# BogdanDIA/gr-dvbt

Hardware: AMD Instinct MI355X
Metric: RX Msamples/s (baseband in -> TS out) (higher is better)
Workload: dtype u8 (Viterbi/RS) + f32 (front end)

## Files before the change

gr_dvbt_amd/csrc/k_backend.hpp:

```cpp
#pragma once
#include <hip/hip_runtime.h>
#include <stdint.h>
#include "k_frontend.hpp"

namespace dvbt {

struct InnerParams { int payload, m, csize; int nlev; float inv_step, guard; float hshift; int hier; };
__device__ __forceinline__ float hier_unshift(float x, float hshift) { return copysignf(fmaxf(fabsf(x) - hshift, 0.f), x); }

__device__ __forceinline__ int demap_all(float2 v, const float2 *pts, int csize)
{
  float dr = v.x - pts[0].x, di = v.y - pts[0].y;
  float best = dr * dr + di * di; int idx = 0;
  for (int j = 1; j < csize; j++) {
    dr = v.x - pts[j].x; di = v.y - pts[j].y;
    float d = dr * dr + di * di;
    if (d < best) { best = d; idx = j; }
  }
  return idx;
}

__device__ __forceinline__ int demap_fast(float2 v, const float2 *pts, const unsigned char *label_of, const InnerParams &p)
{
  const bool in_range = p.nlev != 0 && fabsf(v.x) < p.guard && fabsf(v.y) < p.guard;
// ... 60 lines not shown
    const uint8_t *bb = v + blk * 132;
    auto bit = [&](int f) -> int { const int e = f / 126, j = f - e * 126; int w = j - offs[e]; if (w < 0) w += 126; return (bb[w] >> (m - 1 - e)) & 1; };
    const int t0 = m * i;
    const int hp = (bit((t0 & 1) * 126 + t0 / 2) << 1) | bit(((t0 + 1) & 1) * 126 + (t0 + 1) / 2);
    int lp = 0;
    for (int k = 2; k < m - 2; k++) {
      const int t = t0 + k, e = (t % (m - 2)) / ((m - 2) / 2) + 2 * (t % ((m - 2) / 2)) + 2, f = e * 126 + t / (m - 2);
      lp = (lp << 1) | (f < m * 126 ? bit(f) : 0);
    }
    o_hp[idx] = (uint8_t)hp;
    if (o_lp) o_lp[idx] = (uint8_t)lp;
  }
}

constexpr int INNER_NB = 12;
constexpr int INNER_THREADS = DVBT_INNER_THREADS;
template <int MODE> __global__ __launch_bounds__(INNER_THREADS) void inner_kernel(const float2 *__restrict__ eq, const uint8_t *__restrict__ in_bytes, InnerParams p,
                                                   const RxState *st, int nitems_fixed, const int *__restrict__ sym_index,
                                                   const float2 *__restrict__ points, const unsigned char *__restrict__ label_tab,
                                                   const uint16_t *__restrict__ H, const uint16_t *__restrict__ Hinv,
                                                   uint8_t *__restrict__ tap_demap, uint8_t *__restrict__ tap_symdeint,
                                                   uint8_t *__restrict__ out, uint8_t *__restrict__ out_lp = nullptr)
{
  extern __shared__ __attribute__((aligned(16))) unsigned char smem_raw[];
  uint8_t *v = smem_raw;
  float2 *pts = reinterpret_cast<float2 *>(smem_raw + ((((p.payload + IB - 1) / IB) * IBS + 15) & ~15));
  unsigned char *label_of = reinterpret_cast<unsigned char *>(pts + 64);
  const int u = blockIdx.x, tid = threadIdx.x;
  constexpr int mode = MODE;
  int first = 0, nout = nitems_fixed;
  if (st) { first = st->first_out; nout = st->n_out_symbols; if (first < 0) return; }
  if (u >= nout) return;
  const int s = first + u;
  if (mode & 1) {
    for (int j = tid; j < p.csize; j += INNER_THREADS) pts[j] = points[j];
    if (tid < 64) label_of[tid] = label_tab[tid];
  }
  __syncthreads();
  const bool odd = (mode & 2) ? (sym_index[s] & 1) : false;
  const float2 *e = eq ? eq + (size_t)s * p.payload : nullptr;
  const uint8_t *ib = in_bytes ? in_bytes + (size_t)s * p.payload : nullptr;
  const uint16_t *ptab = odd ? H : Hinv;
  for (int q0 = tid; q0 < p.payload; q0 += INNER_NB * INNER_THREADS) {
    unsigned pk[INNER_NB];
#pragma unroll
    for (int k = 0; k < INNER_NB; k++) {
      const int q = q0 + k * INNER_THREADS, qc = q < p.payload ? q : p.payload - 1;
      pk[k] = (mode & 2) ? (unsigned)ptab[qc] : (unsigned)qc;
      if (!(mode & 1)) pk[k] |= (unsigned)ib[qc] << 16;
    }
#pragma unroll
    for (int k = 0; k < INNER_NB; k++) {
      const int q = q0 + k * INNER_THREADS;
      if (q < p.payload) {
        const int lab = (mode & 1) ? demap_one(e[q], pts, label_of, p) : (int)(pk[k] >> 16);
        const int dst = (int)(pk[k] & 0xffffu);
        const int blk = dst / IB, r = dst - blk * IB, at = blk * IBS + r;
        v[at] = (uint8_t)lab;
        if (r < IBS - IB) v[at + IB] = (uint8_t)lab;
        if (tap_demap && (mode & 1)) tap_demap[(size_t)u * p.payload + q] = (uint8_t)lab;
      }
    }
  }
  __syncthreads();
  uint8_t *o = out + (size_t)u * p.payload;
  if (tap_symdeint) for (int q = tid; q < p.payload; q += INNER_THREADS) tap_symdeint[(size_t)u * p.payload + q] = v[ipos(q)];
  if (!(mode & 4)) { for (int q = tid; q < p.payload; q += INNER_THREADS) o[q] = v[ipos(q)]; return; }
  if (p.hier) bit_deint_hier(v, o, out_lp ? out_lp + (size_t)u * p.payload : nullptr, p.payload, p.m, tid);
  else if (p.m == 2) bit_deint_words<2>(v, o, p.payload, tid);
  else if (p.m == 4) bit_deint_words<4>(v, o, p.payload, tid);
  else bit_deint_words<6>(v, o, p.payload, tid);
}

struct VitParams {
  int m, k, n, plen, ntb, bsize;
  int d_nsymbols;
  int d_nbits;
  int chunk_bytes;
  int payload;
  unsigned punct_mask;
  int warm;
  unsigned long long prefix_nib;
  unsigned long long magic_plen, magic_m;
  unsigned long long punct_rep;
  unsigned magic16_plen;
  uint8_t punct[16], prefix[16];
};

__device__ __forceinline__ void plan_body(RxState *st, const VitParams &vp, long long sym_off)
{
  const long long ibits = (long long)vp.payload * vp.m * vp.k / vp.n;
  const long long nin_g = (sym_off + (long long)st->n_out_symbols) * vp.payload;
  const long long nblocks_g = nin_g / vp.d_nsymbols;
  long long nin = nblocks_g * vp.d_nsymbols - sym_off * vp.payload;
  long long steps = nblocks_g * (vp.d_nbits / 2) - sym_off * ibits;
  if (nin < 0 || steps < 0) { nin = 0; steps = 0; }
  st->n_vit_in = nin;
  st->n_vit_steps = steps;
  long long nb_g = nblocks_g * (vp.d_nbits / 2) / 8 - vp.ntb;
  if (nb_g < 0) nb_g = 0;
  long long nb = steps / 8 - vp.ntb;
  if (nb < 0) nb = 0;
  st->n_vit_bytes = nb;
  const long long items_g = (nb_g / 1632) & ~1ll;
  long long words = items_g * 8 - sym_off * ibits / (8 * 204);
  if (words < 0) words = 0;
  st->stream_rs_items = items_g;
  st->n_rs_words = words;
  st->n_rs_items = words / 8;
  st->sym_off = sym_off;
  st->n_ts_bytes = 0; st->rs_fail = 0; st->rs_corr = 0; st->ts_first_packet = 0; st->rs_list_n = 0;
}
__global__ __launch_bounds__(256) void tps_tail_kernel(FrontParams p, RxState *st, const SymInfo *info, const int *maj, TpsState *ts, int *sym_index,
                                                      const TpsEdge *edges, const int *first_cand, int *need_seq, int clear_d_init, VitParams vp, long long sym_off)
{
  int seq = 1;
  if (edges) seq = tps_finalize_body(st, edges, first_cand, need_seq, p.keep_last, ts);
  if (seq) tps_fsm_body(p, st, 0, info, maj, ts, sym_index, (int *)nullptr, (const unsigned char *)nullptr, clear_d_init);
  if (threadIdx.x == 0) plan_body(st, vp, sym_off);
}

struct RsTables { const uint8_t *div_tab;  const uint8_t *gexp;  const uint8_t *glog;  };

constexpr int RS_SYN_STRIDE = 65;
__device__ inline int rs_decode_word_wave(uint8_t *cw, const uint8_t *syn, const uint8_t *gexp, const uint8_t *glog,
                                          int compat, uint8_t *scr, int lane)
{
  auto gmul = [&](int a, int b) -> int { return (a == 0 || b == 0) ? 0 : gexp[glog[a] + glog[b]]; };
  auto gdiv = [&](int a, int b) -> int { return (a == 0 || b == 0) ? 0 : gexp[255 + glog[a] - glog[b]]; };
  auto wxor = [&](int v) -> int { for (int o = 16; o > 0; o >>= 1) v ^= __shfl_xor(v, o); return v; };
  int sig = lane == 0 ? 1 : 0, bb = sig, el = 0;
  for (int r = 1; r <= 16; r++) {
    int term = (lane < r && lane <= 16) ? gmul(sig, syn[(r - 1 - lane) * RS_SYN_STRIDE]) : 0;
    const int discr = __shfl(wxor(term), 0);
    int bup = __shfl_up(bb, 1); if (lane == 0) bup = 0;
    if (discr == 0) bb = bup;
    else {
      const int T = sig ^ gmul(discr, bup);
      if (2 * el <= r - 1) { el = r - el; bb = gdiv(sig, discr); } else bb = bup;
      sig = lane <= 16 ? T : 0;
    }
  }
  const unsigned long long nz = __ballot(sig != 0 && lane <= 16);
  const int deg_sigma = nz ? 63 - __clzll(nz) : 0;
  uint8_t *s_sig = scr, *s_root = scr + 17, *s_om = scr + 34;
  if (lane <= 16) s_sig[lane] = (uint8_t)sig;
  __builtin_amdgcn_fence(__ATOMIC_SEQ_CST, "wavefront");
  int found[4]; int nroots = 0;
  unsigned long long bal[4];
  for (int k = 0; k < 4; k++) {
    const int i = lane + 1 + 64 * k;
    int q = 1;
    if (i <= 255) {
      for (int j = 1; j <= deg_sigma; j++) { int sg = s_sig[j]; if (sg) q ^= gexp[(glog[sg] + (j * i) % 255) % 255]; }
    }
    found[k] = (i <= 255) && (q == 0);
    bal[k] = __ballot(found[k]);
  }
  {
    int before = 0;
    for (int k = 0; k < 4; k++) {
      if (found[k]) { int rank = before + __popcll(bal[k] & ((1ull << lane) - 1)); if (rank < 17 && rank < deg_sigma) s_root[rank] = (uint8_t)(lane + 1 + 64 * k); }
      before += __popcll(bal[k]);
    }
    nroots = before < deg_sigma ? before : deg_sigma;
  }
// ... 410 lines not shown
```

gr_dvbt_amd/csrc/k_viterbi3.hpp:

```cpp
#pragma once
#include <hip/hip_runtime.h>
#include <stdint.h>
#include <limits.h>
#include <string.h>
#include "dvbt_tables.hpp"
#include "k_backend.hpp"

namespace dvbt {

inline VitParams make_vit_params(const Dims &d, int bsize, int chunk_bytes)
{
  VitParams v; memset(&v, 0, sizeof v);
  v.m = d.m; v.k = d.k; v.n = d.n; v.plen = d.plen; v.ntb = d.ntb; v.bsize = bsize;
  v.d_nsymbols = bsize * d.n / d.m; v.d_nbits = 2 * d.k * bsize;
  v.chunk_bytes = chunk_bytes > 0 ? chunk_bytes : 768; v.payload = d.payload; v.warm = 72;
  memcpy(v.punct, d.punct, 16); memcpy(v.prefix, d.prefix, 16);
  v.punct_mask = 0; v.prefix_nib = 0;
  for (int i = 0; i < d.plen; i++) { v.punct_mask |= (unsigned)d.punct[i] << i; v.prefix_nib |= (unsigned long long)d.prefix[i] << (4 * i); }
  v.magic_plen = ~0ull / (unsigned)d.plen + 1; v.magic_m = ~0ull / (unsigned)d.m + 1;
  for (int i = 0; i < 64; i++) v.punct_rep |= (unsigned long long)d.punct[i % d.plen] << i;
  v.magic16_plen = (65536u + (unsigned)d.plen - 1) / (unsigned)d.plen;
  return v;
}

#define DPP_XOR1 0xB1
#define DPP_XOR2 0x4E
#define DPP_HALF_MIRROR 0x141
#define DPP_ROR8 0x128
#define DPP_MIRROR 0x140

__device__ __forceinline__ int rotl6(int c, int p) { return ((c << p) | (c >> (6 - p))) & 63; }

#ifndef V3_WGW_N
#define V3_WGW_N 4
#endif
constexpr int V3_WGW = V3_WGW_N;
#ifndef V3_EXP
#define V3_EXP 0
#endif
constexpr int V3_WARM = 72;
constexpr int V3_WARM_MAX = 1152;
static_assert(V3_WARM == 72, "make_vit_params (above) presets VitParams.warm to the default");
constexpr int V3_BLK = 24;
constexpr int V3_RENORM_EVERY = 6;
constexpr int V3_RENORM_BEST = -72;
static_assert(V3_BLK % V3_RENORM_EVERY == 0, "a block of windows ends right behind a renormalisation: equal states are equal registers at a block's top (proof, repair, carried state)");
static_assert(V3_RENORM_BEST % 2 == 0, "the renormalisation leaves bit 8 of the cells alone");
static_assert(V3_RENORM_BEST - 49 - 4 >= -128, "lowest candidate of a step: the best field never decreases, the spread is at most 49, |delta| <= 4");
static_assert(V3_RENORM_BEST + 1 + 4 * 8 * V3_RENORM_EVERY + 4 <= 127, "highest candidate of a step: the best field rises by at most 4 per step, 8 steps per window");
constexpr int V3_RINGW = 64;
constexpr int V3_WAVES_PER_CU = 4 * 2;
constexpr int V3_CBW = 17;

typedef short v3pk __attribute__((ext_vector_type(2)));
__device__ __forceinline__ v3pk pk(int x) { return __builtin_bit_cast(v3pk, x); }
__device__ __forceinline__ int ipk(v3pk x) { return __builtin_bit_cast(int, x); }
__device__ __forceinline__ int pk_add(int a, int b) { return ipk(pk(a) + pk(b)); }
__device__ __forceinline__ int pk_sub(int a, int b) { return ipk(pk(a) - pk(b)); }
__device__ __forceinline__ int pk_max(int a, int b) { return ipk(__builtin_elementwise_max(pk(a), pk(b))); }
__device__ __forceinline__ int pk_min(int a, int b) { return ipk(__builtin_elementwise_min(pk(a), pk(b))); }
template <int CTRL> __device__ __forceinline__ int dppb(int v) { return __builtin_amdgcn_update_dpp(0, v, CTRL, 0xf, 0xf, true); }
__device__ __forceinline__ int vconst(int c) { int x; asm("v_mov_b32 %0, %1" : "=v"(x) : "s"(c)); return x; }
__device__ __forceinline__ int pk_max_swap(int a, int b) { int r; asm("v_pk_max_i16 %0, %1, %2 op_sel:[0,1] op_sel_hi:[1,0]" : "=v"(r) : "v"(a), "v"(b)); return r; }
template <bool HI> __device__ __forceinline__ int pk_add_half(int a, int b)
{
  int r;
  if (HI) asm("v_pk_add_u16 %0, %1, %2 op_sel:[0,1] op_sel_hi:[1,1]" : "=v"(r) : "v"(a), "v"(b));
  else asm("v_pk_add_u16 %0, %1, %2 op_sel:[0,0] op_sel_hi:[1,0]" : "=v"(r) : "v"(a), "v"(b));
  return r;
}
template <bool HI> __device__ __forceinline__ int pk_sub_half(int a, int b)
{
  int r;
  if (HI) asm("v_pk_sub_i16 %0, %1, %2 op_sel:[0,1] op_sel_hi:[1,1]" : "=v"(r) : "v"(a), "v"(b));
  else asm("v_pk_sub_i16 %0, %1, %2 op_sel:[0,0] op_sel_hi:[1,0]" : "=v"(r) : "v"(a), "v"(b));
  return r;
}

struct V3Lane {
  unsigned sel[6];
  int bias8[6][2];
  int kc[3][2];
  int org[2];
  int arm_mid[3][2];
  int arm_b2[3][2];
  int arm_org[3][2];
};

__device__ __forceinline__ int v3_phys(int a) { const int a2 = (a >> 2) & 1; return (a & 8) | (a2 << 2) | ((a & 3) ^ (a2 ? 3 : 0)); }
__device__ __forceinline__ int v3_log(int p) { const int q = p & 7, a2 = (q >> 2) & 1; return (p & 8) | (a2 << 2) | ((q ^ (a2 ? 7 : 0)) & 3); }
__device__ __forceinline__ int v3_cell_of_z(int z) { return ((z & 2) << 4) | ((z & 1) << 4) | v3_log(z >> 2); }
__device__ __forceinline__ int v3_z_of_cell(int c) { return v3_phys(c & 15) * 4 + ((c >> 5) & 1) * 2 + ((c >> 4) & 1); }

__device__ __forceinline__ int v3_upper(int P, int r, int h, int a) { const int c = (r << 5) | (h << 4) | a; return (c >> (5 - P)) & 1; }
__device__ __forceinline__ unsigned v3_class(int P, int r, int h, int a)
{
  const int c = (r << 5) | (h << 4) | a, i = rotl6(c, P) & 31;
  const int c0 = ((i >> 2) ^ (i >> 1) ^ i) & 1;
  const int c1 = ((i >> 4) ^ (i >> 2) ^ (i >> 1)) & 1;
  return (unsigned)(c0 | (c1 << 1));
}
__device__ inline void v3_init_lane(int pl, V3Lane &L)
// ... 120 lines not shown
__device__ __forceinline__ void v3_trace_out(const V3Trace &T, const unsigned char *tab, uint8_t *outb) { unsigned t[2]; v3_trace_read(T, tab, t); v3_trace_store<false>(T, t, outb); }

__device__ __forceinline__ void v3_load_words(const unsigned *wp_, unsigned (&W)[8])
{
  const uint4 *wp = reinterpret_cast<const uint4 *>(wp_);
  const uint4 t0 = wp[0], t1 = wp[1];
  W[0] = t0.x; W[1] = t0.y; W[2] = t0.z; W[3] = t0.w; W[4] = t1.x; W[5] = t1.y; W[6] = t1.z; W[7] = t1.w;
}
template <int V6, int W0, bool HOPS, int HOP0, int NTB, int NW, bool PREF> __device__ __forceinline__ void v3_fwd_window(int (&v)[2], const V3Lane &L, const unsigned *wrow, unsigned char *tab, unsigned char *tabw,
                                                                                           unsigned char *bests, int jb, int dd, int pl, V3Trace &T, unsigned (&W)[8], unsigned (&Wn)[8], uint8_t *outb)
{
  constexpr bool HOPA = HOPS && HOP0 + 2 * V6 < NTB - 1, HOPB = HOPS && HOP0 + 2 * V6 + 1 < NTB - 1;
  constexpr bool FINA = HOPS && HOP0 + 2 * V6 == NTB - 1, FINB = HOPS && HOP0 + 2 * V6 + 1 == NTB - 1;
  unsigned th[2], tout[2];
  if (HOPA) v3_hop_read(T, tab, th);
  if (FINA) v3_trace_read(T, tab, tout);
  constexpr int WB = W0 + V6;
  static_assert(V3_BLK % 8 == 0 && V3_RINGW % 8 == 0, "jb % 8 == 0: the ring's wrap falls between two groups of eight windows");
  const int jr = ((jb + (WB & ~7)) & (V3_RINGW - 1)) + (WB & 7);
#if V3_EXP & 256
  for (int i = 0; i < 8; i++) { W[i] = (unsigned)((jb + W0) * 0x01010101 + i * 0x00020406 + pl); asm volatile("" : "+v"(W[i])); }
#else
  if (PREF) v3_load_words(wrow + (V6 + 1) * 8, Wn);
#endif
  constexpr int P0 = (8 * V6) % 6;
  int raw[2];
#if V3_EXP & 32
  if (V6 & 1) __builtin_amdgcn_s_setprio(1); else __builtin_amdgcn_s_setprio(0);
#endif
#if V3_EXP & 128
  __builtin_amdgcn_s_sleep(1);
#endif
  v3_step<(P0 + 0) % 6, 0>(v, W[0], L, raw); V3_YIELD(); v3_step<(P0 + 1) % 6, 0>(v, W[1], L, raw); V3_YIELD(); v3_step<(P0 + 2) % 6, 3>(v, W[2], L, raw); V3_YIELD();
  if (HOPA) { v3_hop_merge<NW>(T, th); if (HOPB) v3_hop_read(T, tab, th); }
  if (FINB) v3_trace_read(T, tab, tout);
  if (FINA) v3_trace_store<true>(T, tout, outb);
  v3_step<(P0 + 3) % 6, 0>(v, W[3], L, raw); V3_YIELD(); v3_step<(P0 + 4) % 6, 0>(v, W[4], L, raw); V3_YIELD(); v3_step<(P0 + 5) % 6, 1>(v, W[5], L, raw); V3_YIELD();
  v3_step<(P0 + 6) % 6, 4>(v, W[6], L, raw); V3_YIELD(); v3_step<(P0 + 7) % 6, 2>(v, W[7], L, raw);
  if (HOPB) v3_hop_merge<NW>(T, th);
  if (FINB) v3_trace_store<true>(T, tout, outb);
  if (!(V3_EXP & 4)) *reinterpret_cast<unsigned *>(tabw + jr * V3_ROW<NW>) = __builtin_amdgcn_perm((unsigned)raw[1], (unsigned)raw[0], 0x06040200u);
  if (V3_EXP & 2) { if (raw[0] == 0x12345) bests[jr] = 1; return; }
  const int s = v3_window_end<(P0 + 2) % 6, V6 == V3_RENORM_EVERY - 1>(v, L);
  bests[dd * V3_RINGW + jr] = (unsigned char)s;
}
static_assert(V3_RENORM_EVERY == 6, "v3_fwd_six is the group of windows that ends in a renormalisation (V6 = 0..5)");
template <int W0, bool HOPS, int HOP0, int NTB, int NW, bool MORE> __device__ __forceinline__ void v3_fwd_six(int (&v)[2], const V3Lane &L, const unsigned *wrow, unsigned char *tab, unsigned char *tabw,
                                                                                  unsigned char *bests, int jb, int dd, int pl, V3Trace &T, unsigned (&Wa)[8], unsigned (&Wb)[8], uint8_t *outb)
{
  v3_fwd_window<0, W0, HOPS, HOP0, NTB, NW, true>(v, L, wrow, tab, tabw, bests, jb, dd, pl, T, Wa, Wb, outb); v3_fwd_window<1, W0, HOPS, HOP0, NTB, NW, true>(v, L, wrow, tab, tabw, bests, jb, dd, pl, T, Wb, Wa, outb);
  v3_fwd_window<2, W0, HOPS, HOP0, NTB, NW, true>(v, L, wrow, tab, tabw, bests, jb, dd, pl, T, Wa, Wb, outb); v3_fwd_window<3, W0, HOPS, HOP0, NTB, NW, true>(v, L, wrow, tab, tabw, bests, jb, dd, pl, T, Wb, Wa, outb);
  v3_fwd_window<4, W0, HOPS, HOP0, NTB, NW, true>(v, L, wrow, tab, tabw, bests, jb, dd, pl, T, Wa, Wb, outb); v3_fwd_window<5, W0, HOPS, HOP0, NTB, NW, MORE>(v, L, wrow, tab, tabw, bests, jb, dd, pl, T, Wb, Wa, outb);
}

#if V3_EXP & 16
__device__ unsigned long long *v3_dbg;
#endif

constexpr int V3_SLOT = 32;
constexpr int V3_CTL_CHUNKS = 0;
constexpr int V3_CTL_MISMATCH = 1;
constexpr int V3_CTL_CONFLICT = 2;
constexpr int V3_CTL_UNPROVEN = 3;
constexpr int V3_CTL_SEQ = 4;
constexpr int V3_CTL_ACC = 8;
constexpr int V3_CTL_SHORT = 12;
constexpr int V3_CTL_HDR = 16;
struct V3Aux {
  int *snap;
  int *ctl;
  long long cap;
  long long grid0;
  const int *carry_in;
  int *carry_out; int carry_rel;
  int debug;
};
constexpr int V3_DEBUG_WALK = 2;
__device__ __forceinline__ int *v3_own(const V3Aux &ax, long long c) { return ax.snap + (3 * c) * V3_SLOT; }
__device__ __forceinline__ int *v3_pred(const V3Aux &ax, long long c) { return ax.snap + (3 * c + 1) * V3_SLOT; }
__device__ __forceinline__ int *v3_fix(const V3Aux &ax, long long c) { return ax.snap + (3 * c + 2) * V3_SLOT; }
inline size_t v3_snap_words(long long cap) { return (size_t)(cap + 2) * 3 * V3_SLOT; }
inline size_t v3_ctl_words(long long cap) { return (size_t)V3_CTL_HDR + 2 * (size_t)(cap + 2); }

struct V3Lds { unsigned char *tab; unsigned *wbuf; unsigned char *bests; const unsigned *lut; int wv; };
__device__ __forceinline__ void v3_init_lut(unsigned *lut, int lane)
{
  if (lane < 16) {
    const int k0 = (lane >> 2) & 1, k1 = (lane >> 3) & 1, t1 = (lane >> 1) & 1, t0 = lane & 1;
    const int u0 = k0 ? 1 - 2 * t1 : 0, u1 = k1 ? 1 - 2 * (k0 ? t0 : t1) : 0;
    const unsigned d0 = (unsigned)(2 * (u0 + u1)) & 0xff, d1 = (unsigned)(2 * (-u0 + u1)) & 0xff;
    const unsigned d2 = (unsigned)(2 * (u0 - u1)) & 0xff, d3 = (unsigned)(2 * (-u0 - u1)) & 0xff;
    lut[lane] = d0 | (d1 << 8) | (d2 << 16) | (d3 << 24);
  }
}

template <int NTB, int WARM, int MODE, int NW>
__device__ __forceinline__ void v3_decode(const uint8_t *__restrict__ in, uint8_t *__restrict__ out, long long total_steps, long long total_out, const VitParams &vp,
                                          long long in_base, long long out_lo, long long b0, bool dec_active, const V3Lds &S, const V3Lane &L, int (&v)[2], int (&endv)[2],
                                          int *own, int *predn, const int *inject, int *carry, int carry_rel, int debug, unsigned long long *shortcut)
{
  unsigned char *const tab = S.tab; unsigned *const wbuf = S.wbuf; unsigned char *const bests = S.bests; const unsigned *const lut = S.lut;
  unsigned *const cbits = wbuf;
  constexpr int V3_CBS = V3_BLK * 8;
  static_assert(V3_CBW <= V3_CBS, "bit stream does not fit the step-word row");
  const int lane = threadIdx.x & 63, dd = lane >> 4, pl = lane & 15;
  const int rowl = S.wv * 256 + dd * 64;
  unsigned char *const tabw = tab + rowl + pl * 4;
  const int B = vp.chunk_bytes, m = vp.m;
  constexpr int ntb = NTB;
  const long long b1 = (b0 + B < total_out) ? b0 + B : total_out;
  const int warm = MODE == 2 ? 0 : WARM > 0 ? WARM : vp.warm;
  const long long w0 = b0 + 2 - warm;
  const int J = ((warm + B + ntb - 1 + V3_BLK - 1) / V3_BLK) * V3_BLK;
  const long long n_in_bytes = (total_steps * 2 / vp.plen * vp.n + vp.m - 1) / vp.m;
  const int nload = ((384 + 2 * m - 2) / m + 3 + 15) / 16;

  uint8_t *const outb = out + (b0 - out_lo);
  const int ob_end = !dec_active ? INT_MIN : (int)(b1 - b0 > INT_MIN / 2 ? b1 - b0 : INT_MIN / 2);
  const int ob_lo = MODE != 1 || out_lo <= b0 ? 0 : (int)(out_lo - b0 < INT_MAX / 2 ? out_lo - b0 : INT_MAX / 2);
  const long long tb0 = 8 * (w0 - 1) - 2;
  constexpr int BLKBITS = 2 * 8 * V3_BLK;
  const int inc_q = BLKBITS / vp.plen, inc_ph = BLKBITS - inc_q * vp.plen;
  const unsigned magic16_m = (65536u + (unsigned)m - 1) / (unsigned)m;

  int u_first, u_last;
  {
    const long long r = total_steps - 8 * V3_BLK - tb0;
    int first = tb0 >= 0 ? 0 : (int)((-tb0 + 7) >> 3 < J ? (-tb0 + 7) >> 3 : J), last = !dec_active || r < 0 ? -1 : (int)(r >> 3 < J ? r >> 3 : J);
    u_first = max(max(__builtin_amdgcn_readlane(first, 0), __builtin_amdgcn_readlane(first, 16)), max(__builtin_amdgcn_readlane(first, 32), __builtin_amdgcn_readlane(first, 48)));
    u_last = min(min(__builtin_amdgcn_readlane(last, 0), __builtin_amdgcn_readlane(last, 16)), min(__builtin_amdgcn_readlane(last, 32), __builtin_amdgcn_readlane(last, 48)));
  }
  auto pfx = [&](int ph) { return (int)__popc(vp.punct_mask & ((1u << ph) - 1u)); };
  int ph0 = 0, pf0 = 0, bo0 = 0, off = 0; long long byte0 = 0; uint4 q = make_uint4(0, 0, 0, 0);
  auto stage_load = [&](int jb) {
    const long long tb = tb0 + (long long)jb * 8;
    if (jb > 0 && jb - V3_BLK >= u_first) {
      const int pf_old = pf0;
      ph0 += inc_ph;
      const int wrap = ph0 >= vp.plen ? 1 : 0;
      ph0 -= wrap ? vp.plen : 0;
      pf0 = pfx(ph0);
      const int r = bo0 + (inc_q + wrap) * vp.n + pf0 - pf_old;
      const int dby = (int)(((unsigned)r * magic16_m) >> 16);
      bo0 = r - dby * m; byte0 += dby;
    } else {
      const unsigned long long pbit = 2ull * (unsigned long long)(tb > 0 ? tb : 0);
      const unsigned long long pq = __umul64hi(pbit, vp.magic_plen);
      ph0 = (int)(pbit - pq * (unsigned)vp.plen); pf0 = pfx(ph0);
      const unsigned long long rb = pq * (unsigned)vp.n + (unsigned)pf0;
      const unsigned long long by = __umul64hi(rb, vp.magic_m);
      byte0 = (long long)by; bo0 = (int)(rb - by * (unsigned)m);
    }
    off = (int)(((unsigned long long)(uintptr_t)in + (unsigned long long)(byte0 - in_base)) & 3ull);
    const long long src = byte0 - off + pl * 16;
    q = make_uint4(0, 0, 0, 0);
    if (dec_active && pl < nload) {
      if (src >= in_base && src + 16 <= n_in_bytes) q = *reinterpret_cast<const uint4 *>(in + (src - in_base));
      else {
        unsigned w[4] = {0, 0, 0, 0};
        for (int i = 0; i < 16; i++) {
          const long long bb = src + i;
          const unsigned bv = (bb >= in_base && bb < n_in_bytes) ? in[bb - in_base] : 0;
          w[i >> 2] |= bv << (8 * (i & 3));
        }
        q = make_uint4(w[0], w[1], w[2], w[3]);
      }
    }
  };
  auto stage_words = [&](int jb, auto &&mid) {
    {
      const unsigned mk = (1u << m) - 1;
      auto grp = [&](unsigned d) { return ((d & mk) << (3 * m)) | (((d >> 8) & mk) << (2 * m)) | (((d >> 16) & mk) << m) | ((d >> 24) & mk); };
      const unsigned g0 = grp(q.x), g1 = grp(q.y), g2 = grp(q.z), g3 = grp(q.w);
      unsigned *cb = cbits + dd * V3_CBS;
      if (pl < nload) {
        if (m == 2) cb[pl] = (g0 << 24) | (g1 << 16) | (g2 << 8) | g3;
        else if (m == 4) { cb[2 * pl] = (g0 << 16) | g1; cb[2 * pl + 1] = (g2 << 16) | g3; }
        else { cb[3 * pl] = (g0 << 8) | (g1 >> 16); cb[3 * pl + 1] = (g1 << 16) | (g2 >> 8); cb[3 * pl + 2] = (g2 << 24) | g3; }
      }
    }
    __builtin_amdgcn_fence(__ATOMIC_SEQ_CST, "wavefront");
    constexpr int SPL = V3_BLK * 8 / 16;
    const long long tb = tb0 + (long long)jb * 8;
    const int ub0 = pl * SPL;
    int lo = 0, hi = SPL;
    int x = ph0 + 2 * ub0;
    if (jb < u_first || jb > u_last) {
      const long long tbr = tb > 0 ? tb : 0;
      const long long t = tb + ub0;
      if (t < 0) lo = (-t < SPL) ? (int)(-t) : SPL;
      const long long rem = total_steps - t;
      hi = !dec_active ? 0 : rem <= 0 ? 0 : rem < SPL ? (int)rem : SPL;
      if (hi < lo) hi = lo;
      x = ph0 + 2 * (int)((t + lo) - tbr);
      if (x < 0) x = 0;
    }
    const int dq = (int)(((unsigned)x * vp.magic16_plen) >> 16);
    const int ph = x - dq * vp.plen;
    const int pos = off * m + bo0 + dq * vp.n + pfx(ph) - pf0;
    const unsigned kmask = ((unsigned)(vp.punct_rep >> ph) << (2 * lo)) & (((1u << (2 * hi)) - 1u) & ~((1u << (2 * lo)) - 1u));
    const unsigned *cb = cbits + dd * V3_CBS;
    const unsigned cw0 = cb[pos >> 5], cw1 = cb[(pos >> 5) + 1];
    mid();
    unsigned win = (unsigned)(((((unsigned long long)cw0) << 32) | cw1) >> (32 - (pos & 31)));
    unsigned idx[SPL], sw[SPL];
#pragma unroll
    for (int i = 0; i < SPL; i++) {
      const unsigned k2 = (kmask >> (2 * i)) & 3u;
      idx[i] = (k2 << 2) | (win >> 30);
      win <<= __popc(k2);
    }
#pragma unroll
    for (int i = 0; i < SPL; i++) sw[i] = lut[idx[i]];
    static_assert(SPL % 4 == 0, "a lane's step words are whole 16-byte groups (its offset dd * 768 + pl * 48 bytes is 16-byte aligned)");
    uint4 *const wdst = reinterpret_cast<uint4 *>(wbuf + dd * (V3_BLK * 8) + ub0);
#pragma unroll
    for (int i = 0; i < SPL / 4; i++) wdst[i] = make_uint4(sw[4 * i], sw[4 * i + 1], sw[4 * i + 2], sw[4 * i + 3]);
    __builtin_amdgcn_fence(__ATOMIC_SEQ_CST, "wavefront");
  };
  V3Trace T;
  int tsh[2];
  int tsh_e[2];
#pragma unroll
  for (int c = 0; c < 2; c++) {
    tsh_e[c] = (2 * ((c * 16 + pl + 1 + 3 * ntb - (ntb - 1)) % 3) + 4) % 6;
    T.oend[c] = c * 16 + pl < V3_BLK ? ob_end : INT_MIN; tsh[c] = (2 * ((c * 16 + pl + 1) % 3) + 4) % 6; T.osh[c] = (6 - 2 * ((c * 16 + pl + 3 * ntb - (ntb - 1)) % 3)) % 6;
  }
  static_assert(V3_BLK % 3 == 0, "phases per lane");
  auto bests_read = [&](int jp, unsigned (&bb)[2]) {
#pragma unroll
    for (int c = 0; c < 2; c++) bb[c] = bests[dd * V3_RINGW + ((jp + c * 16 + pl) & (V3_RINGW - 1))];
  };
  auto z_of_best = [](unsigned b, int sh) { const unsigned R = (b | (b << 6)) >> sh; return (R ^ 51u ^ (((R >> 4) & 1u) * 12u)) & 63u; };
  auto trace_init = [&](int jp, const unsigned (&bb)[2]) {
#pragma unroll
    for (int c = 0; c < 2; c++) {
      const int jj = jp + c * 16 + pl;
      T.ob[c] = jj - (warm + ntb - 1);
      T.ok[c] = __builtin_amdgcn_ballot_w64(T.ob[c] >= ob_lo && T.ob[c] < T.oend[c]);
      T.wsh[c] = jj * V3_ROW<NW> + rowl;
      T.z[c] = (int)z_of_best(bb[c], tsh[c]) | (T.wsh[c] & V3_RMASK<NW>);
    }
  };
  unsigned bb[2], be[2], tl[2], te[2];
  int zp[2], zcarry = 0;
  auto bests_read_ends = [&](int jp) {
#pragma unroll
    for (int c = 0; c < 2; c++) be[c] = bests[dd * V3_RINGW + ((jp + c * 16 + pl - (ntb - 1)) & (V3_RINGW - 1))];
  };
  auto link_reads = [&](int jp) {
    trace_init(jp, bb);
    zp[0] = __builtin_amdgcn_update_dpp(zcarry, T.z[0], 0x111, 0xf, 0xf, false);
    zp[1] = __builtin_amdgcn_update_dpp(dppb<0x121>(T.z[0]), T.z[1], 0x111, 0xf, 0xf, false);
#pragma unroll
    for (int c = 0; c < 2; c++) tl[c] = tab[T.z[c]];
    zcarry = dppb<0x129>(T.z[1]);
  };
  auto end_reads = [&]() {
#pragma unroll
    for (int c = 0; c < 2; c++) te[c] = tab[(int)z_of_best(be[c], tsh_e[c]) | ((T.wsh[c] - (ntb - 1) * V3_ROW<NW>) & V3_RMASK<NW>)];
  };
  auto links_hold = [&](int jp) {
    const bool fails = jp - (warm + ntb - 1) < ob_end && ((((tl[0] ^ (unsigned)zp[0]) & 63u) != 0) || (pl < V3_BLK - 16 && ((tl[1] ^ (unsigned)zp[1]) & 63u) != 0));
    return __builtin_amdgcn_ballot_w64(fails) == 0;
  };
  bool ok_prev = false;
  unsigned n_short = 0, n_walk = 0;

  stage_load(0);
  for (int jb = 0; jb < J; jb += V3_BLK) {
    if (MODE == 1 && dec_active) {
      if (jb == warm) { if (inject) { v[0] = inject[0]; v[1] = inject[1]; } own[0] = v[0]; own[1] = v[1]; }
      if (jb == warm + B) { predn[0] = v[0]; predn[1] = v[1]; }
      if (carry && jb == warm + carry_rel) { carry[0] = v[0]; carry[1] = v[1]; }
    }
    if (MODE == 2) {
      if (jb == 0 && dec_active) { own[0] = v[0]; own[1] = v[1]; }
      if (jb == B) { endv[0] = v[0]; endv[1] = v[1]; }
      if (carry && dec_active && jb == carry_rel) { carry[0] = v[0]; carry[1] = v[1]; }
    }
    bests_read(jb - V3_BLK, bb);
    bests_read_ends(jb - V3_BLK);
    if (!(V3_EXP & 8) || jb == 0) stage_words(jb, [&]() { link_reads(jb - V3_BLK); });
    else link_reads(jb - V3_BLK);
    if (jb + V3_BLK < J && !(V3_EXP & 8)) stage_load(jb + V3_BLK);
    const bool ok_cur = jb > 0 && links_hold(jb - V3_BLK);
    const bool ends = (T.ok[0] | T.ok[1]) != 0;
    const bool fast = ok_cur && ok_prev && !(debug & V3_DEBUG_WALK) && !(V3_EXP & 1);
    ok_prev = ok_cur;
    const bool tr = jb > 0 && !fast && ends && !(V3_EXP & 1);
    if (fast && ends) { end_reads(); v3_trace_store<true>(T, te, outb); n_short++; }
    if (tr) n_walk++;
    const unsigned *wrow = wbuf + dd * (V3_BLK * 8);
    unsigned Wa[8], Wb[8];
    v3_load_words(wrow, Wa);
    if (tr) {
      v3_fwd_six<0, true, 0, NTB, NW, true>(v, L, wrow, tab, tabw, bests, jb, dd, pl, T, Wa, Wb, outb);
      v3_fwd_six<6, true, 12, NTB, NW, true>(v, L, wrow + 48, tab, tabw, bests, jb, dd, pl, T, Wa, Wb, outb);
    } else {
      v3_fwd_six<0, false, 0, NTB, NW, true>(v, L, wrow, tab, tabw, bests, jb, dd, pl, T, Wa, Wb, outb);
      v3_fwd_six<6, false, 0, NTB, NW, true>(v, L, wrow + 48, tab, tabw, bests, jb, dd, pl, T, Wa, Wb, outb);
    }
    static_assert(V3_BLK == 24, "the second half of the block is written out: two groups of six windows, straight-line like the first half");
    static_assert(NTB - 1 < 24, "the chains' last read takes a hop slot of the first twelve windows");
    v3_fwd_six<12, false, 0, NTB, NW, true>(v, L, wrow + 96, tab, tabw, bests, jb, dd, pl, T, Wa, Wb, outb);
    v3_fwd_six<18, false, 0, NTB, NW, false>(v, L, wrow + 144, tab, tabw, bests, jb, dd, pl, T, Wa, Wb, outb);
  }
  __builtin_amdgcn_fence(__ATOMIC_SEQ_CST, "wavefront");
  bests_read(J - V3_BLK, bb);
  trace_init(J - V3_BLK, bb);
  for (int h = 0; h < ntb - 1; h++) v3_hop<NW>(T, tab);
  v3_trace_out(T, tab, outb);
  if (MODE == 1 && shortcut && lane == 0) { atomicAdd(shortcut, (unsigned long long)n_short); atomicAdd(shortcut + 1, (unsigned long long)n_walk); }
}

template <int NW> struct V3Shared {
  alignas(16) unsigned char tab[V3_RINGW * V3_ROW<NW>];
  alignas(16) unsigned wbuf[NW][4 * V3_BLK * 8];
  unsigned char bests[NW][4 * V3_RINGW];
  unsigned lut[16];
};
static_assert(sizeof(V3Shared<4>) <= 81920 && V3_RMASK<4> == 0xffc0 && V3_RMASK<1> == 0x3fc0, "two four-wave workgroups per CU beside the symbol kernel's 76 KB");
#define V3_LDS_DECL(NW) __shared__ V3Shared<NW> sh_;
#define V3_LDS(NW, wv) V3Lds{sh_.tab, sh_.wbuf[wv], sh_.bests[wv], sh_.lut, wv}

template <int NTB, int WARM = V3_WARM, int MODE = 0> __global__ __launch_bounds__(64 * V3_WGW) void viterbi3_kernel(const uint8_t *__restrict__ in, uint8_t *__restrict__ out, const RxState *st,
                                                      long long steps_fixed, VitParams vp, V3Aux ax, long long in_base, long long out_lo)
{
  V3_LDS_DECL(V3_WGW)
  const int wv = V3_WGW > 1 ? (int)(threadIdx.x >> 6) : 0;
  const V3Lds S = V3_LDS(V3_WGW, wv);
  const int lane = threadIdx.x & 63, dd = lane >> 4, pl = lane & 15;
  const long long total_steps = st ? st->n_vit_steps : steps_fixed;
  const long long total_out = total_steps / 8 - vp.ntb;
  const int B = vp.chunk_bytes;
  if (MODE == 1 && blockIdx.x == 0 && threadIdx.x == 0) {
    ax.ctl[V3_CTL_MISMATCH] = 0; ax.ctl[V3_CTL_CONFLICT] = 0; ax.ctl[V3_CTL_UNPROVEN] = -1; ax.ctl[V3_CTL_SEQ] = 0;
  }
  const long long grid0 = MODE == 1 ? ax.grid0 : out_lo;
  const long long chunk0 = ((long long)blockIdx.x * V3_WGW + wv) * 4;
  if (grid0 + chunk0 * B >= total_out) return;
  const long long c = chunk0 + dd, b0 = grid0 + c * B;
  const bool dec_active = b0 < total_out;
  v3_init_lut(sh_.lut, lane);
#if V3_EXP & 16
  const unsigned long long dbg_t0 = wall_clock64();
#endif
  V3Lane L; v3_init_lane(pl, L);
  constexpr int v3_start = (int)(((unsigned)(V3_RENORM_BEST & 0xff) << 8) * 0x00010001u);
  int v[2] = {L.arm_org[0][0] | v3_start, L.arm_org[0][1] | v3_start}, endv[2];
  int *own = nullptr, *predn = nullptr, *carry = nullptr; const int *inject = nullptr;
  if (MODE == 1) {
    own = v3_own(ax, c) + 2 * pl; predn = v3_pred(ax, c + 1) + 2 * pl;
    if (c == 0 && ax.carry_in) inject = ax.carry_in + 2 * pl;
    if (ax.carry_out && b0 + B >= total_out) carry = ax.carry_out + 2 * pl;
  }
  v3_decode<NTB, WARM, MODE, V3_WGW>(in, out, total_steps, total_out, vp, in_base, out_lo, b0, dec_active, S, L, v, endv, own, predn, inject, carry, ax.carry_rel, ax.debug,
                                     MODE == 1 ? reinterpret_cast<unsigned long long *>(ax.ctl + V3_CTL_SHORT) : nullptr);
#if V3_EXP & 16
  if (lane == 0) {
    unsigned id, xcc;
    asm volatile("s_getreg_b32 %0, hwreg(HW_REG_HW_ID)" : "=s"(id));
    asm volatile("s_getreg_b32 %0, hwreg(HW_REG_XCC_ID)" : "=s"(xcc));
    unsigned long long *d = v3_dbg + 3 * ((long long)blockIdx.x * V3_WGW + wv);
    d[0] = (id & 0xffffu) | ((xcc & 0xfu) << 16); d[1] = dbg_t0; d[2] = wall_clock64();
  }
#endif
}

__device__ __forceinline__ long long v3_nchunks(long long total_out, long long grid0, int B) { return total_out > grid0 ? (total_out - grid0 + B - 1) / B : 0; }
__device__ __forceinline__ bool v3_slots_equal(const int *a_, const int *b_)
{
  const int4 *a = reinterpret_cast<const int4 *>(a_), *b = reinterpret_cast<const int4 *>(b_);
  bool same = true;
#pragma unroll
  for (int i = 0; i < 8; i++) { const int4 x = a[i], y = b[i]; same = same && x.x == y.x && x.y == y.y && x.z == y.z && x.w == y.w; }
  return same;
}

__global__ __launch_bounds__(256) void viterbi_check_kernel(V3Aux ax, const RxState *st, long long steps_fixed, VitParams vp, int pass)
{
  const long long total_steps = st ? st->n_vit_steps : steps_fixed;
  const long long nch = v3_nchunks(total_steps / 8 - vp.ntb, ax.grid0, vp.chunk_bytes);
  if (blockIdx.x == 0 && threadIdx.x == 0) { ax.ctl[V3_CTL_CHUNKS] = (int)(nch < INT_MAX ? nch : INT_MAX); if (pass == 1) ax.ctl[V3_CTL_UNPROVEN] = 0; }
  const long long c = (long long)blockIdx.x * 256 + threadIdx.x + 1;
  if (c >= nch || c > ax.cap) return;
  const bool same = v3_slots_equal(v3_own(ax, c), v3_pred(ax, c));
  if (pass == 0) {
    ax.ctl[V3_CTL_HDR + (ax.cap + 2) + c] = 0;
    if (!same) ax.ctl[V3_CTL_HDR + atomicAdd(ax.ctl + V3_CTL_MISMATCH, 1)] = (int)c;
  }
}
__global__ __launch_bounds__(256) void viterbi_count_kernel(V3Aux ax, const RxState *st, long long steps_fixed, VitParams vp)
{
  const long long total_steps = st ? st->n_vit_steps : steps_fixed;
  const long long nch = v3_nchunks(total_steps / 8 - vp.ntb, ax.grid0, vp.chunk_bytes);
  const long long c = (long long)blockIdx.x * 256 + threadIdx.x + 1;
  if (c >= nch || c > ax.cap) return;
  if (!v3_slots_equal(v3_own(ax, c), v3_pred(ax, c))) atomicAdd(ax.ctl + V3_CTL_UNPROVEN, 1);
}

__device__ __forceinline__ bool v3_row_equal(const int (&a)[2], const int (&b)[2], int dd)
{
  const unsigned long long ne = __ballot(a[0] != b[0] || a[1] != b[1]);
// ... 121 lines not shown
```

Baseline: 40030.

## Pair step-word LUT lookups, add bounds-free fast input loads, compact depuncture bits

Widens the LDS step-word table from 16 single entries to 256 pair entries, so each lookup yields two step words and halves the index and LDS read work per lane. Precomputes the block range whose 16-byte input loads are always in bounds, so those blocks skip the per-load bound checks and the byte-wise fallback. The edge path clamps byte bounds once instead of testing each byte. It also replaces the per-byte symbol-bit grouping with a shift-mask compaction and tracks the input pointer directly. In exchange the table takes 2 KB of LDS, leaving the shared struct just under the two-workgroups-per-CU limit.

New measurement: 40800, median of 6. 1.9% higher.

```diff
diff --git a/gr_dvbt_amd/csrc/k_backend.hpp b/gr_dvbt_amd/csrc/k_backend.hpp
--- a/gr_dvbt_amd/csrc/k_backend.hpp
+++ b/gr_dvbt_amd/csrc/k_backend.hpp
@@ -166,6 +166,7 @@
   int warm;
   unsigned long long prefix_nib;
   unsigned long long magic_plen, magic_m;
+  unsigned long long magic_n;
   unsigned long long punct_rep;
   unsigned magic16_plen;
   uint8_t punct[16], prefix[16];
diff --git a/gr_dvbt_amd/csrc/k_viterbi3.hpp b/gr_dvbt_amd/csrc/k_viterbi3.hpp
--- a/gr_dvbt_amd/csrc/k_viterbi3.hpp
+++ b/gr_dvbt_amd/csrc/k_viterbi3.hpp
@@ -17,7 +17,7 @@
   memcpy(v.punct, d.punct, 16); memcpy(v.prefix, d.prefix, 16);
   v.punct_mask = 0; v.prefix_nib = 0;
   for (int i = 0; i < d.plen; i++) { v.punct_mask |= (unsigned)d.punct[i] << i; v.prefix_nib |= (unsigned long long)d.prefix[i] << (4 * i); }
-  v.magic_plen = ~0ull / (unsigned)d.plen + 1; v.magic_m = ~0ull / (unsigned)d.m + 1;
+  v.magic_plen = ~0ull / (unsigned)d.plen + 1; v.magic_m = ~0ull / (unsigned)d.m + 1; v.magic_n = ~0ull / (unsigned)d.n + 1;
   for (int i = 0; i < 64; i++) v.punct_rep |= (unsigned long long)d.punct[i % d.plen] << i;
   v.magic16_plen = (65536u + (unsigned)d.plen - 1) / (unsigned)d.plen;
   return v;
@@ -304,16 +304,37 @@
 inline size_t v3_snap_words(long long cap) { return (size_t)(cap + 2) * 3 * V3_SLOT; }
 inline size_t v3_ctl_words(long long cap) { return (size_t)V3_CTL_HDR + 2 * (size_t)(cap + 2); }
 
-struct V3Lds { unsigned char *tab; unsigned *wbuf; unsigned char *bests; const unsigned *lut; int wv; };
-__device__ __forceinline__ void v3_init_lut(unsigned *lut, int lane)
-{
-  if (lane < 16) {
-    const int k0 = (lane >> 2) & 1, k1 = (lane >> 3) & 1, t1 = (lane >> 1) & 1, t0 = lane & 1;
-    const int u0 = k0 ? 1 - 2 * t1 : 0, u1 = k1 ? 1 - 2 * (k0 ? t0 : t1) : 0;
-    const unsigned d0 = (unsigned)(2 * (u0 + u1)) & 0xff, d1 = (unsigned)(2 * (-u0 + u1)) & 0xff;
-    const unsigned d2 = (unsigned)(2 * (u0 - u1)) & 0xff, d3 = (unsigned)(2 * (-u0 - u1)) & 0xff;
-    lut[lane] = d0 | (d1 << 8) | (d2 << 16) | (d3 << 24);
-  }
+struct V3Lds { unsigned char *tab; unsigned *wbuf; unsigned char *bests; const uint2 *lut; int wv; };
+__device__ __forceinline__ unsigned v3_step_word(int e)
+{
+  const int k0 = (e >> 2) & 1, k1 = (e >> 3) & 1, t1 = (e >> 1) & 1, t0 = e & 1;
+  const int u0 = k0 ? 1 - 2 * t1 : 0, u1 = k1 ? 1 - 2 * (k0 ? t0 : t1) : 0;
+  const unsigned d0 = (unsigned)(2 * (u0 + u1)) & 0xff, d1 = (unsigned)(2 * (-u0 + u1)) & 0xff;
+  const unsigned d2 = (unsigned)(2 * (u0 - u1)) & 0xff, d3 = (unsigned)(2 * (-u0 - u1)) & 0xff;
+  return d0 | (d1 << 8) | (d2 << 16) | (d3 << 24);
+}
+constexpr int V3_PAIRS = 256;
+__device__ __forceinline__ void v3_init_lut(uint2 *lut, int lane)
+{
+#pragma unroll
+  for (int j = 0; j < V3_PAIRS / 64; j++) {
+    const int e = lane + 64 * j, k4 = e >> 4, t = e & 15;
+    const int used = __popc(k4 & 3);
+    lut[e] = make_uint2(v3_step_word(((k4 & 3) << 2) | (t >> 2)), v3_step_word((k4 & 12) | (((t << used) >> 2) & 3)));
+  }
+}
+
+template <int M> __device__ __forceinline__ unsigned v3_compact(unsigned d)
+{
+  constexpr unsigned c2 = ((1u << M) - 1) * 0x00010001u;
+  const unsigned t = ((d & c2) << M) | ((d >> 8) & c2);
+  return ((t & ((1u << (2 * M)) - 1)) << (2 * M)) | (t >> 16);
+}
+typedef unsigned v3u4 __attribute__((ext_vector_type(4)));
+__device__ __forceinline__ uint4 v3_load16(unsigned long long addr)
+{
+  const v3u4 t = *(const __attribute__((address_space(1))) v3u4 *)addr;
+  return make_uint4(t.x, t.y, t.z, t.w);
 }
 
 template <int NTB, int WARM, int MODE, int NW>
@@ -321,7 +342,7 @@
                                           long long in_base, long long out_lo, long long b0, bool dec_active, const V3Lds &S, const V3Lane &L, int (&v)[2], int (&endv)[2],
                                           int *own, int *predn, const int *inject, int *carry, int carry_rel, int debug, unsigned long long *shortcut)
 {
-  unsigned char *const tab = S.tab; unsigned *const wbuf = S.wbuf; unsigned char *const bests = S.bests; const unsigned *const lut = S.lut;
+  unsigned char *const tab = S.tab; unsigned *const wbuf = S.wbuf; unsigned char *const bests = S.bests; const uint2 *const lut = S.lut;
   unsigned *const cbits = wbuf;
   constexpr int V3_CBS = V3_BLK * 8;
   static_assert(V3_CBW <= V3_CBS, "bit stream does not fit the step-word row");
@@ -352,8 +373,33 @@
     u_first = max(max(__builtin_amdgcn_readlane(first, 0), __builtin_amdgcn_readlane(first, 16)), max(__builtin_amdgcn_readlane(first, 32), __builtin_amdgcn_readlane(first, 48)));
     u_last = min(min(__builtin_amdgcn_readlane(last, 0), __builtin_amdgcn_readlane(last, 16)), min(__builtin_amdgcn_readlane(last, 32), __builtin_amdgcn_readlane(last, 48)));
   }
+  const unsigned long long in_addr = (unsigned long long)(uintptr_t)in;
+  const int ld_lanes = dec_active ? nload : 0;
+  int l_first, l_last;
+  {
+    const int a = (int)(in_addr & 3ull);
+    const long long H = n_in_bytes - in_base + a - 16 * nload;
+    const long long Rlo = (in_base + ((4 - a) & 3)) * m;
+    const long long Rhi = (in_base + (H & ~3ll) + 3 - a + 1) * m - 1;
+    int first = 0, last = J;
+    if (dec_active) {
+      if (Rlo > 0) {
+        const unsigned long long p = (__umul64hi((unsigned long long)(Rlo - 1), vp.magic_n) + 1) * (unsigned)vp.plen;
+        const long long w = ((long long)((p + 1) >> 1) - tb0 + 7) >> 3;
+        first = w <= 0 ? 0 : w >= J ? J : (((int)w + V3_BLK - 1) / V3_BLK) * V3_BLK;
+      }
+      if (H < 0 || Rhi < 0) last = -1;
+      else {
+        const unsigned long long p = __umul64hi((unsigned long long)Rhi, vp.magic_n) * (unsigned)vp.plen;
+        const long long w = ((long long)(p >> 1) - tb0) >> 3;
+        last = w < 0 ? -1 : w >= J ? J : ((int)w / V3_BLK) * V3_BLK;
+      }
+    }
+    l_first = max(max(__builtin_amdgcn_readlane(first, 0), __builtin_amdgcn_readlane(first, 16)), max(__builtin_amdgcn_readlane(first, 32), __builtin_amdgcn_readlane(first, 48)));
+    l_last = min(min(__builtin_amdgcn_readlane(last, 0), __builtin_amdgcn_readlane(last, 16)), min(__builtin_amdgcn_readlane(last, 32), __builtin_amdgcn_readlane(last, 48)));
+  }
   auto pfx = [&](int ph) { return (int)__popc(vp.punct_mask & ((1u << ph) - 1u)); };
-  int ph0 = 0, pf0 = 0, bo0 = 0, off = 0; long long byte0 = 0; uint4 q = make_uint4(0, 0, 0, 0);
+  int ph0 = 0, pf0 = 0, bo0 = 0, off = 0; unsigned long long pb = 0; uint4 q = make_uint4(0, 0, 0, 0);
   auto stage_load = [&](int jb) {
     const long long tb = tb0 + (long long)jb * 8;
     if (jb > 0 && jb - V3_BLK >= u_first) {
@@ -364,25 +410,30 @@
       pf0 = pfx(ph0);
       const int r = bo0 + (inc_q + wrap) * vp.n + pf0 - pf_old;
       const int dby = (int)(((unsigned)r * magic16_m) >> 16);
-      bo0 = r - dby * m; byte0 += dby;
+      bo0 = r - dby * m; pb += (unsigned)dby;
     } else {
       const unsigned long long pbit = 2ull * (unsigned long long)(tb > 0 ? tb : 0);
       const unsigned long long pq = __umul64hi(pbit, vp.magic_plen);
       ph0 = (int)(pbit - pq * (unsigned)vp.plen); pf0 = pfx(ph0);
       const unsigned long long rb = pq * (unsigned)vp.n + (unsigned)pf0;
       const unsigned long long by = __umul64hi(rb, vp.magic_m);
-      byte0 = (long long)by; bo0 = (int)(rb - by * (unsigned)m);
-    }
-    off = (int)(((unsigned long long)(uintptr_t)in + (unsigned long long)(byte0 - in_base)) & 3ull);
-    const long long src = byte0 - off + pl * 16;
+      pb = in_addr + (by - (unsigned long long)in_base); bo0 = (int)(rb - by * (unsigned)m);
+    }
+    off = (int)((unsigned)pb & 3u);
+    const unsigned long long la = (pb & ~3ull) + (unsigned)(pl * 16);
     q = make_uint4(0, 0, 0, 0);
-    if (dec_active && pl < nload) {
-      if (src >= in_base && src + 16 <= n_in_bytes) q = *reinterpret_cast<const uint4 *>(in + (src - in_base));
+    if (__builtin_expect(jb >= l_first && jb <= l_last, 1)) {
+      if (pl < ld_lanes) q = v3_load16(la);
+    } else if (pl < ld_lanes) {
+      const long long src = (long long)(la - in_addr) + in_base;
+      if (src >= in_base && src + 16 <= n_in_bytes) q = v3_load16(la);
       else {
+        const long long d0 = in_base - src, d1 = n_in_bytes - src;
+        const int e0 = d0 < 0 ? 0 : d0 > 16 ? 16 : (int)d0, e1 = d1 < 0 ? 0 : d1 > 16 ? 16 : (int)d1;
+        const uint8_t *const pbyte = in + (src - in_base);
         unsigned w[4] = {0, 0, 0, 0};
         for (int i = 0; i < 16; i++) {
-          const long long bb = src + i;
-          const unsigned bv = (bb >= in_base && bb < n_in_bytes) ? in[bb - in_base] : 0;
+          const unsigned bv = (i >= e0 && i < e1) ? pbyte[i] : 0;
           w[i >> 2] |= bv << (8 * (i & 3));
         }
         q = make_uint4(w[0], w[1], w[2], w[3]);
@@ -391,14 +442,14 @@
   };
   auto stage_words = [&](int jb, auto &&mid) {
     {
-      const unsigned mk = (1u << m) - 1;
-      auto grp = [&](unsigned d) { return ((d & mk) << (3 * m)) | (((d >> 8) & mk) << (2 * m)) | (((d >> 16) & mk) << m) | ((d >> 24) & mk); };
-      const unsigned g0 = grp(q.x), g1 = grp(q.y), g2 = grp(q.z), g3 = grp(q.w);
       unsigned *cb = cbits + dd * V3_CBS;
       if (pl < nload) {
-        if (m == 2) cb[pl] = (g0 << 24) | (g1 << 16) | (g2 << 8) | g3;
-        else if (m == 4) { cb[2 * pl] = (g0 << 16) | g1; cb[2 * pl + 1] = (g2 << 16) | g3; }
-        else { cb[3 * pl] = (g0 << 8) | (g1 >> 16); cb[3 * pl + 1] = (g1 << 16) | (g2 >> 8); cb[3 * pl + 2] = (g2 << 24) | g3; }
+        if (m == 2) cb[pl] = (v3_compact<2>(q.x) << 24) | (v3_compact<2>(q.y) << 16) | (v3_compact<2>(q.z) << 8) | v3_compact<2>(q.w);
+        else if (m == 4) { cb[2 * pl] = (v3_compact<4>(q.x) << 16) | v3_compact<4>(q.y); cb[2 * pl + 1] = (v3_compact<4>(q.z) << 16) | v3_compact<4>(q.w); }
+        else {
+          const unsigned g0 = v3_compact<6>(q.x), g1 = v3_compact<6>(q.y), g2 = v3_compact<6>(q.z), g3 = v3_compact<6>(q.w);
+          cb[3 * pl] = (g0 << 8) | (g1 >> 16); cb[3 * pl + 1] = (g1 << 16) | (g2 >> 8); cb[3 * pl + 2] = (g2 << 24) | g3;
+        }
       }
     }
     __builtin_amdgcn_fence(__ATOMIC_SEQ_CST, "wavefront");
@@ -425,15 +476,15 @@
     const unsigned cw0 = cb[pos >> 5], cw1 = cb[(pos >> 5) + 1];
     mid();
     unsigned win = (unsigned)(((((unsigned long long)cw0) << 32) | cw1) >> (32 - (pos & 31)));
-    unsigned idx[SPL], sw[SPL];
-#pragma unroll
-    for (int i = 0; i < SPL; i++) {
-      const unsigned k2 = (kmask >> (2 * i)) & 3u;
-      idx[i] = (k2 << 2) | (win >> 30);
-      win <<= __popc(k2);
-    }
-#pragma unroll
-    for (int i = 0; i < SPL; i++) sw[i] = lut[idx[i]];
+    unsigned idx[SPL / 2], sw[SPL];
+#pragma unroll
+    for (int i = 0; i < SPL / 2; i++) {
+      const unsigned k4 = (kmask >> (4 * i)) & 15u;
+      idx[i] = (k4 << 4) | (win >> 28);
+      win <<= __popc(k4);
+    }
+#pragma unroll
+    for (int i = 0; i < SPL / 2; i++) { const uint2 w2 = lut[idx[i]]; sw[2 * i] = w2.x; sw[2 * i + 1] = w2.y; }
     static_assert(SPL % 4 == 0, "a lane's step words are whole 16-byte groups (its offset dd * 768 + pl * 48 bytes is 16-byte aligned)");
     uint4 *const wdst = reinterpret_cast<uint4 *>(wbuf + dd * (V3_BLK * 8) + ub0);
 #pragma unroll
@@ -540,8 +591,9 @@
   alignas(16) unsigned char tab[V3_RINGW * V3_ROW<NW>];
   alignas(16) unsigned wbuf[NW][4 * V3_BLK * 8];
   unsigned char bests[NW][4 * V3_RINGW];
-  unsigned lut[16];
+  uint2 lut[V3_PAIRS];
 };
+static_assert(sizeof(V3Shared<4>) == 80896, "79 KiB: two workgroups are 158 of a CU's 160 KiB");
 static_assert(sizeof(V3Shared<4>) <= 81920 && V3_RMASK<4> == 0xffc0 && V3_RMASK<1> == 0x3fc0, "two four-wave workgroups per CU beside the symbol kernel's 76 KB");
 #define V3_LDS_DECL(NW) __shared__ V3Shared<NW> sh_;
 #define V3_LDS(NW, wv) V3Lds{sh_.tab, sh_.wbuf[wv], sh_.bests[wv], sh_.lut, wv}
```
